# ndefilippis/SWRaytracing

Measured on AMD Instinct MI355X. Metric: packet-steps/sec @ 512² field, 1e6 packets; 1/2/4/8-GPU scaling, higher is better.
Workload: dtype f64

## Files before the change

### swraytracing_amd/csrc/swrt_bin.hpp

```cpp
#pragma once
#include <hip/hip_runtime.h>
#include <stdint.h>

#include "swrt_kernels.hpp"

namespace swrt {

struct BinGeom {
  double dx, px, py, inv_px, inv_py, inv_dx;
  int nx;
  int tile;
  int ntx;
};

__device__ __forceinline__ int tile_of(const BinGeom& g, double x, double y) {
  const int cx = fast_cell(x, g.inv_dx, g.nx);
  const int cy = fast_cell(y, g.inv_dx, g.nx);
  return (cx / g.tile) * g.ntx + (cy / g.tile);
}

constexpr int kMaxBins = 16384;
constexpr int kBinPerThread = 4;

__global__ void __launch_bounds__(256) bin_count_kernel(BinGeom g, const double* x, int64_t n,
                                                        int nbins, int* keys, int* counts) {
  extern __shared__ int hist[];
  for (int b = threadIdx.x; b < nbins; b += blockDim.x) hist[b] = 0;
  __syncthreads();
  const int64_t base = (int64_t)blockIdx.x * blockDim.x * kBinPerThread;
  for (int q = 0; q < kBinPerThread; ++q) {
    const int64_t p = base + (int64_t)q * blockDim.x + threadIdx.x;
    if (p < n) {
      const int key = tile_of(g, x[p], x[n + p]);
      keys[p] = key;
      atomicAdd(&hist[key], 1);
    }
  }
  __syncthreads();
  for (int b = threadIdx.x; b < nbins; b += blockDim.x) {
    const int c = hist[b];
    if (c) atomicAdd(&counts[b], c);
  }
}

constexpr int kOrderBuckets = 16;

__global__ void __launch_bounds__(1024) bin_scan_kernel(int* counts, int nbins, int* cursor,
                                                        int* starts, int64_t n, int* err, int* order = nullptr,
                                                        int lanes = 512) {
  __shared__ int part[1024];
  const int per = (nbins + 1023) / 1024;
  const int b0 = threadIdx.x * per;
  int s = 0;
  int neg = 0;
  for (int i = 0; i < per; ++i) {
    const int b = b0 + i;
    if (b < nbins) {
      const int c = counts[b];
      neg |= c < 0;
      s += c;
    }
  }
  part[threadIdx.x] = s;
  neg = __syncthreads_or(neg);
  for (int off = 1; off < 1024; off <<= 1) {
    const int v = threadIdx.x >= off ? part[threadIdx.x - off] : 0;
    __syncthreads();
    part[threadIdx.x] += v;
    __syncthreads();
  }
  if (neg || (int64_t)part[1023] != n) {
    for (int b = threadIdx.x; b < nbins; b += blockDim.x) {
      cursor[b] = (int)n;
      starts[b] = 0;
      counts[b] = 0;
    }
    if (threadIdx.x == 0) {
      starts[nbins] = 0;
      __hip_atomic_store(err, 1, __ATOMIC_RELAXED, __HIP_MEMORY_SCOPE_SYSTEM);
    }
    if (order != nullptr)
      for (int b = threadIdx.x; b < nbins; b += blockDim.x) order[b] = b;
    return;
  }
  int run = threadIdx.x ? part[threadIdx.x - 1] : 0;
  for (int i = 0; i < per; ++i) {
    const int b = b0 + i;
    if (b < nbins) {
      cursor[b] = run;
      starts[b] = run;
      run += counts[b];
      counts[b] = 0;
    }
  }
  if (threadIdx.x == 1023) starts[nbins] = part[1023];
  if (order == nullptr) return;
  __syncthreads();
  const int wave = threadIdx.x >> 6, lane = threadIdx.x & 63;
  if (nbins % 8 != 0) {
    for (int b = threadIdx.x; b < nbins; b += blockDim.x) order[b] = b;
    return;
  }
  if (wave >= 8) return;
  const int tpx = nbins / 8, base = wave * tpx;
  const uint64_t below = (1ull << lane) - 1;
  int cnt[kOrderBuckets];
#pragma unroll
  for (int v = 0; v < kOrderBuckets; ++v) cnt[v] = 0;
  for (int c0 = 0; c0 < tpx; c0 += 64) {
    const int i = c0 + lane;
    const int r = i < tpx ? min((starts[base + i + 1] - starts[base + i] + lanes - 1) / lanes, kOrderBuckets - 1) : -1;
#pragma unroll
    for (int v = 0; v < kOrderBuckets; ++v) cnt[v] += __popcll(__ballot(r == v));
  }
  int acc = 0;
#pragma unroll
  for (int v = kOrderBuckets - 1; v >= 0; --v) {
    const int c = cnt[v];
    cnt[v] = acc;
    acc += c;
  }
  for (int c0 = 0; c0 < tpx; c0 += 64) {
    const int i = c0 + lane;
    const int r = i < tpx ? min((starts[base + i + 1] - starts[base + i] + lanes - 1) / lanes, kOrderBuckets - 1) : -1;
#pragma unroll
    for (int v = 0; v < kOrderBuckets; ++v) {
      const uint64_t m = __ballot(r == v);
      if (r == v) order[base + cnt[v] + __popcll(m & below)] = base + i;
      cnt[v] += __popcll(m);
    }
  }
}

template <bool INDEX>
__global__ void __launch_bounds__(256) bin_scatter_kernel(const double* x, const double* k,
                                                          const int* perm, const int* keys, int64_t n,
                                                          int nbins, int* cursor, double* x2,
                                                          double* k2, int* perm2, int* src) {
  extern __shared__ int sh[];
  int* cnt = sh;
  int* base = sh + nbins;
  for (int b = threadIdx.x; b < nbins; b += blockDim.x) cnt[b] = 0;
  __syncthreads();
  const int64_t b0 = (int64_t)blockIdx.x * blockDim.x * kBinPerThread;
  int key[kBinPerThread], local[kBinPerThread];
#pragma unroll
  for (int q = 0; q < kBinPerThread; ++q) {
    const int64_t p = b0 + (int64_t)q * blockDim.x + threadIdx.x;
    key[q] = 0;
    local[q] = 0;
    if (p < n) {
      key[q] = keys[p];
      local[q] = atomicAdd(&cnt[key[q]], 1);
    }
  }
  __syncthreads();
  for (int b = threadIdx.x; b < nbins; b += blockDim.x) {
    const int c = cnt[b];
    if (c) base[b] = atomicAdd(&cursor[b], c);
  }
  __syncthreads();
#pragma unroll
  for (int q = 0; q < kBinPerThread; ++q) {
    const int64_t p = b0 + (int64_t)q * blockDim.x + threadIdx.x;
    if (p < n) {
      const int64_t d = (int64_t)base[key[q]] + local[q];
      if (d < 0 || d >= n) continue;
      if constexpr (INDEX) {
        src[d] = (int)p;
        continue;
      }
      x2[d] = x[p];
      x2[n + d] = x[n + p];
      k2[d] = k[p];
      k2[n + d] = k[n + p];
      perm2[d] = perm[p];
    }
  }
}

__global__ void iota_kernel(int* perm, int64_t n) {
  const int64_t p = (int64_t)blockIdx.x * blockDim.x + threadIdx.x;
  if (p < n) perm[p] = (int)p;
}

__global__ void unpermute_kernel(const double* x, const double* k, const int* perm, int64_t n, int64_t ld,
                                 double* xo, double* ko) {
  const int64_t p = (int64_t)blockIdx.x * blockDim.x + threadIdx.x;
  if (p >= n) return;
  const int64_t d = perm[p];
  xo[d] = x[p];
  xo[ld + d] = x[n + p];
  ko[d] = k[p];
  ko[ld + d] = k[n + p];
}

}
```

### swraytracing_amd/csrc/swrt_host_fields.hpp

```cpp
#pragma once
#include <vector>

#include "swrt_ctx.hpp"
#include "swrt_fft.hpp"
#include "swrt_kernels.hpp"
#include "swrt_xka.hpp"

namespace {

int ensure_scratch(swrt_ctx* c, size_t bytes) {
  if (c->scratch_bytes >= bytes) return SWRT_OK;
  c->scratch_bytes = 0;
  HIPCHK(c, c->scratch.alloc(bytes));
  c->scratch_bytes = bytes;
  return SWRT_OK;
}

int ensure_twiddles(swrt_ctx* c, int n) {
  if (c->tw_n == n) return SWRT_OK;
  if (c->tw) HIPCHK(c, hipDeviceSynchronize());
  std::vector<double2> h(n);
  for (int k = 0; k < n; ++k) {
    const long double th = -2.0L * 3.14159265358979323846264338327950288L * (long double)k / (long double)n;
    h[k] = make_double2((double)cosl(th), (double)sinl(th));
  }
  HIPCHK(c, c->tw.alloc(n));
  HIPCHK(c, hipMemcpyAsync(c->tw.get(), h.data(), sizeof(double2) * n, hipMemcpyHostToDevice,
                           c->stream));
  HIPCHK(c, hipStreamSynchronize(c->stream));
  c->tw_n = n;
  return SWRT_OK;
}

int ensure_slot(swrt_ctx* c, int slot, int64_t nx) {
  Slot& s = c->slot[slot];
  const int64_t npad = nx + kPadTot;
  if (s.nodes.get() && s.nx == nx) return SWRT_OK;
  if (s.nodes) HIPCHK(c, hipDeviceSynchronize());
  s.psi.reset();
  s.set = false;
  HIPCHK(c, s.nodes.alloc(kRec * npad * npad));
  s.nx = nx;
  s.npad = npad;
  return SWRT_OK;
}

int check_slot_args(swrt_ctx* c, int slot, int64_t nx) {
  if (!c) return SWRT_ERR_ARG;
  if (slot < 0 || slot >= SWRT_MAX_SLOTS) return fail(c, SWRT_ERR_ARG, "slot out of range");
  if (nx < 8 || nx > 4096 || (nx & 1)) return fail(c, SWRT_ERR_ARG, "nx must be even, 8..4096");
  return SWRT_OK;
}

FieldView view_of(const Slot& s) {
  FieldView v;
  v.nodes = s.nodes.get();
  v.nx = (int)s.nx;
  v.npad = (int)s.npad;
  v.dx = s.L / (double)s.nx;
  v.px = (double)s.nx;
  v.py = (double)s.ny_period;
  v.inv_px = 1.0 / v.px;
  v.inv_py = 1.0 / v.py;
  v.ipx = (int)s.nx;
  v.ipy = (int)s.ny_period;
  v.inv_dx = 1.0 / v.dx;
  return v;
}

int pack_slot(swrt_ctx* c, int slot, const double* dplanes, double shear) {
  Slot& s = c->slot[slot];
  const int64_t tot = s.npad * s.npad;
  hipLaunchKernelGGL(pack_nodes_kernel, dim3(nblocks(tot, 256)), dim3(256), 0, c->stream, dplanes,
                     (int)s.nx, (int)s.npad, shear, s.nodes.get());
  HIPCHK(c, hipGetLastError());
  return SWRT_OK;
}

int fft_group(const swrt_ctx* c, int n, int nvec, bool tin) {
  const int C = (c->qg_sep && c->n > 0) ? 1 : 2;
  if (C * (n / 4) > 1024 || nvec % (tin ? 8 * C : C) != 0) return 1;
  return C;
}

template <bool TIN>
void launch_fft(swrt_ctx* c, const double2* in, double2* out, int n, int logn, int nvec, int inverse) {
  if (n <= 1024) {
    const int C = fft_group(c, n, nvec, TIN);
    hipLaunchKernelGGL((fft_vec_kernel<TIN, 2>), dim3((unsigned)(nvec / C)), dim3(C * n / 4),
                       sizeof(double2) * C * (n + 1), c->stream, in, out, n, logn, c->tw.get(), inverse, nvec);
  } else
    hipLaunchKernelGGL((fft_vec_kernel<TIN, 1>), dim3((unsigned)nvec), dim3(128), sizeof(double2) * 2 * n, c->stream,
                       in, out, n, logn, c->tw.get(), inverse, nvec);
}

int run_fft_pass(swrt_ctx* c, double2* Z, int n, int nb, int inverse) {
  const int logn = ilog2(n);
  const int64_t nvec = (int64_t)n * nb;
  launch_fft<false>(c, Z, Z, n, logn, (int)nvec, inverse);
  HIPCHK(c, hipGetLastError());
  return SWRT_OK;
}

int run_transpose(swrt_ctx* c, const double2* in, double2* out, int n, int nb) {
  dim3 grid((n + 31) / 32, (n + 31) / 32, nb);
  hipLaunchKernelGGL(transpose_kernel, grid, dim3(32, 8), 0, c->stream, in, out, n);
  HIPCHK(c, hipGetLastError());
  return SWRT_OK;
}

int transform_2d(swrt_ctx* c, double2* Z, double2* out, int n, int nb, int inverse) {
  int rc;
  if ((rc = run_fft_pass(c, Z, n, nb, inverse))) return rc;
  const int64_t nvec = (int64_t)n * nb;
  if (nvec % 8) {
    if ((rc = run_transpose(c, Z, out, n, nb))) return rc;
    return run_fft_pass(c, out, n, nb, inverse);
  }
  const int logn = ilog2(n);
  launch_fft<true>(c, Z, out, n, logn, (int)nvec, inverse);
  HIPCHK(c, hipGetLastError());
  return SWRT_OK;
}

int inverse_2d(swrt_ctx* c, double2* Z, double2* out, int n, int nb) { return transform_2d(c, Z, out, n, nb, 1); }

int fields_from_halfplane(swrt_ctx* c, int slot, const double2* dfk, int n, int mode, double K_d2,
                          double kscale, double shear, int with_psi, double2* Z, double2* T, int sx, int sy) {
  int rc;
  const int64_t nn = (int64_t)n * n;
  const int nb = with_psi ? 4 : 3;
  Slot& s0 = c->slot[slot];
  if (!with_psi && n % 16 == 0 && 3 * 2 * n / 4 <= 1024 && (n / 2) % 8 == 0) {
    const int logn = ilog2(n);
    hipLaunchKernelGGL(spectra_rows_kernel, dim3((unsigned)n), dim3(3 * n / 4), sizeof(double2) * 3 * n, c->stream,
                       dfk, n, mode, K_d2, kscale, 0, sx, sy, logn, (const double2*)c->tw.get(), Z);
    HIPCHK(c, hipGetLastError());
    hipLaunchKernelGGL(fft_cols_pack_kernel<2>, dim3((unsigned)(n / 2)), dim3(3 * 2 * n / 4),
                       sizeof(double2) * 3 * 2 * (n + 1), c->stream, (const double2*)Z, n, logn,
                       (const double2*)c->tw.get(), (int)s0.npad, shear, s0.nodes.get());
    HIPCHK(c, hipGetLastError());
    s0.has_psi = false;
    s0.div_free = true;
    return SWRT_OK;
  }
  if (nb * n / 4 <= 1024 && ((int64_t)n * nb) % 8 == 0) {
    const int logn = ilog2(n);
    hipLaunchKernelGGL(spectra_rows_kernel, dim3((unsigned)n), dim3(nb * n / 4), sizeof(double2) * nb * n, c->stream,
                       dfk, n, mode, K_d2, kscale, with_psi, sx, sy, logn, (const double2*)c->tw.get(), Z);
    HIPCHK(c, hipGetLastError());
    launch_fft<true>(c, Z, T, n, logn, n * nb, 1);
    HIPCHK(c, hipGetLastError());
  } else {
    hipLaunchKernelGGL(spectra_kernel, dim3(nblocks(nn, 256)), dim3(256), 0, c->stream, dfk, n, mode,
                       K_d2, kscale, with_psi, Z, sx, sy);
    HIPCHK(c, hipGetLastError());
    if ((rc = inverse_2d(c, Z, T, n, nb))) return rc;
  }
  Slot& s = c->slot[slot];
  if (with_psi && !s.psi) HIPCHK(c, s.psi.alloc(nn));
  if (n % 16 == 0) {
    hipLaunchKernelGGL(pack_pairs_kernel, dim3(n / 16, n / 16), dim3(256), 0, c->stream, T, n, (int)s.npad, shear,
                       s.nodes.get());
    HIPCHK(c, hipGetLastError());
    if (with_psi) {
      hipLaunchKernelGGL(psi_plane_kernel, dim3(nblocks(nn, 256)), dim3(256), 0, c->stream, T + 3 * nn, s.psi.get(),
                         nn);
      HIPCHK(c, hipGetLastError());
    }
  } else {
    double* planes = reinterpret_cast<double*>(Z);
    hipLaunchKernelGGL(unpair_kernel, dim3(nblocks(nn, 256)), dim3(256), 0, c->stream, T, n, with_psi,
                       planes, with_psi ? s.psi.get() : nullptr);
    HIPCHK(c, hipGetLastError());
    if ((rc = pack_slot(c, slot, planes, shear))) return rc;
  }
  s.has_psi = with_psi != 0;
  s.div_free = true;
  return SWRT_OK;
}

struct FftScratch {
  double2 *Z, *T, *fk;
  double* raw;
};
FftScratch fft_scratch(swrt_ctx* c, size_t zb, int64_t nhalf) {
  char* base = c->scratch.get();
  return {(double2*)base, (double2*)(base + zb), (double2*)(base + 2 * zb),
          (double*)(base + 2 * zb + sizeof(double2) * nhalf)};
}

int g2k_launches(swrt_ctx* c, const double* raw, double2* Z, double2* T, double2* fk, int n) {
  const int64_t nn = (int64_t)n * n, nhalf = (int64_t)(n - 1) * (n / 2);
  hipLaunchKernelGGL(real_to_complex_kernel, dim3(nblocks(nn, 256)), dim3(256), 0, c->stream, raw, Z, nn);
  HIPCHK(c, hipGetLastError());
  if (int rc = transform_2d(c, Z, T, n, 1, 0)) return rc;
  hipLaunchKernelGGL(crop_half_kernel, dim3(nblocks(nhalf, 256)), dim3(256), 0, c->stream, T, n, fk);
  HIPCHK(c, hipGetLastError());
  return SWRT_OK;
}

int slot_set_done(swrt_ctx* c, int slot, double L, int64_t ny_period) {
  HIPCHK(c, hipStreamSynchronize(c->stream));
  Slot& s = c->slot[slot];
  s.L = L;
  s.ny_period = ny_period;
  s.set = true;
  s.wgen = ++c->slot_wgen;
  return SWRT_OK;
}

int xka_nodes_for(swrt_ctx* c, int64_t nx) {
  const int64_t npad = nx + kPadTot;
  if (c->xka.nx != nx) {
    c->xka.nx = 0;
    HIPCHK(c, c->xka.nodes.alloc(kXkaRec * npad * npad));
    c->xka.nx = nx;
  }
  return SWRT_OK;
}

int xka_pack(swrt_ctx* c, const double* dplanes, int64_t nx) {
  const int64_t npad = nx + kPadTot;
  hipLaunchKernelGGL(pack_xka_kernel, dim3(nblocks(npad * npad, 256)), dim3(256), 0, c->stream, dplanes, (int)nx,
                     (int)npad, c->xka.nodes.get());
  HIPCHK(c, hipGetLastError());
  return SWRT_OK;
}
}
```

### swraytracing_amd/csrc/swrt_kernels.hpp

```cpp
#pragma once
#include <hip/hip_runtime.h>
#include <stdint.h>

#include "swrt_share.hpp"

namespace swrt {

constexpr int kNT = 6;
constexpr int kPadLo = 2;
constexpr int kPadTot = 5;
constexpr int kRec = 6;

struct FieldView {
  const double* nodes;
  int nx;
  int npad;
  double dx;
  double px, py;
  double inv_px, inv_py;
  int ipx, ipy;
  double inv_dx;
};

__device__ __forceinline__ double div_rn(double a, double b, double rb) {
  const double q0 = a * rb;
  const double r = __builtin_fma(-q0, b, a);
  return __builtin_fma(r, rb, q0);
}

__device__ __forceinline__ double div_rn_z(double a, double b, double rb) {
  const double q0 = a * rb;
  const double r = __builtin_fma(q0, b, -a);
  return __builtin_fma(-r, rb, q0);
}

__device__ __forceinline__ double sqrt_rn_normal(double x) {
  const double y = __builtin_amdgcn_rsq(x);
  double g = x * y;
  double h = y * 0.5;
  const double r = __builtin_fma(-h, g, 0.5);
  g = __builtin_fma(g, r, g);
  double d = __builtin_fma(-g, g, x);
  h = __builtin_fma(h, r, h);
  g = __builtin_fma(d, h, g);
  d = __builtin_fma(-g, g, x);
  return __builtin_fma(d, h, g);
}

__device__ __forceinline__ double rcp_rn_normal(double b) {
  double y = __builtin_amdgcn_rcp(b);
  double e = __builtin_fma(-b, y, 1.0);
  y = __builtin_fma(y, e, y);
  e = __builtin_fma(-b, y, 1.0);
  y = __builtin_fma(y, e, y);
  const double r = __builtin_fma(-b, y, 1.0);
  return __builtin_fma(r, y, y);
}

__device__ __forceinline__ void drift_inc(double k, double l, double f2, double gH, double half, bool fast,
                                          double& hcx, double& hcy) {
  const double x = f2 + gH * (k * k + l * l);
  if (fast) {
    const double w = sqrt_rn_normal(x);
    const double rw = rcp_rn_normal(w);
    hcx = half * div_rn_z(gH * k, w, rw);
    hcy = half * div_rn_z(gH * l, w, rw);
  } else {
    const double w = sqrt(x);
    hcx = half * (gH * k / w);
    hcy = half * (gH * l / w);
  }
}

__device__ __forceinline__ void quot2_sqrt(double r, double n1, double n2, bool fast, double& q1, double& q2) {
  if (fast) {
    const double w = sqrt_rn_normal(r);
    const double rw = rcp_rn_normal(w);
    q1 = div_rn_z(n1, w, rw);
    q2 = div_rn_z(n2, w, rw);
  } else {
    const double w = sqrt(r);
    q1 = n1 / w;
    q2 = n2 / w;
  }
}

__host__ __device__ inline bool dispersion_fast(double f2) { return f2 >= 0x1p-767 && f2 < 0x1p+1000; }

__global__ void __launch_bounds__(256) check_arith_kernel(int64_t n, uint64_t seed,
                                                          unsigned long long* mismatches) {
  const int64_t p = (int64_t)blockIdx.x * blockDim.x + threadIdx.x;
  if (p >= n) return;
  uint64_t s = seed ^ (0x9E3779B97F4A7C15ull * (uint64_t)(p + 1));
  auto nxt = [&]() {
    s ^= s << 13; s ^= s >> 7; s ^= s << 17;
    return s;
  };
  auto rnd = [&](int lo, int hi) {
    const uint64_t m = nxt() & ((1ull << 52) - 1);
    const int e = lo + (int)(nxt() % (uint64_t)(hi - lo + 1));
    return __longlong_as_double((long long)(((uint64_t)(e + 1023) << 52) | m));
  };
  unsigned bad[3] = {0, 0, 0};
  for (int it = 0; it < 16; ++it) {
    const double x = rnd(-767, 1023);
    if (__double_as_longlong(sqrt_rn_normal(x)) != __double_as_longlong(sqrt(x))) ++bad[0];
    const double w = rnd(-383, 511);
    if (__double_as_longlong(rcp_rn_normal(w)) != __double_as_longlong(1.0 / w)) ++bad[1];
    const double f2 = rnd(-60, 60), gH = rnd(-30, 30);
    const double k = (nxt() & 1 ? -1.0 : 1.0) * rnd(-40, 40), l = (nxt() & 1 ? -1.0 : 1.0) * rnd(-40, 40);
    double hx, hy, gx, gy;
    drift_inc(k, l, f2, gH, 0.5, true, hx, hy);
    drift_inc(k, l, f2, gH, 0.5, false, gx, gy);
    if (__double_as_longlong(hx) != __double_as_longlong(gx) || __double_as_longlong(hy) != __double_as_longlong(gy))
      ++bad[2];
  }
  for (int q = 0; q < 3; ++q)
    if (bad[q]) atomicAdd(&mismatches[q], (unsigned long long)bad[q]);
}

__device__ __forceinline__ int cvt_i32_sat(double v) {
  int c;
  asm("v_cvt_i32_f64 %0, %1" : "=v"(c) : "v"(v));
  return c;
}

__device__ __forceinline__ int cell_frac(double x, double dx, double inv_dx, double period,
                                         double inv_period, int iperiod, int nx, double& a) {
  const double q = div_rn(x, dx, inv_dx);
  const double r = div_rn(q, period, inv_period);
  const double xl = q - floor(r) * period;
  const double fl = floor(xl);
  a = (1.0 + xl) - (1.0 + fl);
  int c = cvt_i32_sat(fl);
  c = (unsigned)c > (unsigned)iperiod ? 0 : c;
  c = (int)min((unsigned)c, (unsigned)(c - nx));
  c = (int)min((unsigned)c, (unsigned)(c - nx));
  if (iperiod >= 3 * nx) c %= nx;
  return c;
}

template <int D>
__device__ __forceinline__ double div_const(double x) {
  constexpr int A = D < 0 ? -D : D;
  static_assert(A >= 1 && A <= 5, "divisor");
  double q;
  if constexpr (A == 1 || A == 2 || A == 4) {
    q = x * (1.0 / (double)A);
  } else {
    constexpr double R = 1.0 / (double)A;
    const double q0 = x * R;
    const double r = __builtin_fma(-q0, (double)A, x);
    q = __builtin_fma(r, R, q0);
  }
  return D < 0 ? -q : q;
}

constexpr int odd_part(int d) { return d < 0 ? odd_part(-d) : (d % 2 == 0 ? odd_part(d / 2) : d); }
constexpr double pow2_sign_inv(int d) {
  return d < 0 ? -pow2_sign_inv(-d) : (d % 2 == 0 ? 0.5 * pow2_sign_inv(d / 2) : 1.0);
}
template <int I>
constexpr double kScale() {
  double c = 1.0;
  for (int j = -2; j <= 3; ++j)
    if (j != I) c *= pow2_sign_inv(j - I);
  return c;
}

template <int I, int J>
__device__ __forceinline__ double wstep(double w, const double* t) {
  if constexpr (I == J) {
    return w;
  } else {
    return div_const<odd_part(J - I)>(w * t[J + 2]);
  }
}

template <int I>
__device__ __forceinline__ double lagrange_wi(const double* t) {
  double w = 1.0;
  w = wstep<I, -2>(w, t);
  w = wstep<I, -1>(w, t);
  w = wstep<I, 0>(w, t);
  w = wstep<I, 1>(w, t);
  w = wstep<I, 2>(w, t);
  w = wstep<I, 3>(w, t);
  constexpr double S = kScale<I>();
  return S == 1.0 ? w : w * S;
}

__device__ __forceinline__ void lagrange_w(double a, double bump, double w[kNT]) {
  double t[kNT];
#pragma unroll
  for (int j = -2; j <= 3; ++j) t[j + 2] = (a - (double)j) + bump;
  w[0] = lagrange_wi<-2>(t);
  w[1] = lagrange_wi<-1>(t);
  w[2] = lagrange_wi<0>(t);
  w[3] = lagrange_wi<1>(t);
  w[4] = lagrange_wi<2>(t);
  w[5] = lagrange_wi<3>(t);
}

__device__ __forceinline__ int fast_cell(double x, double inv_dx, int nx) {
  const double q = floor(x * inv_dx);
  int c = (q > -1073741824.0 && q < 1073741824.0) ? (int)q : 0;
  c %= nx;
  return c < 0 ? c + nx : c;
}

struct Stencil {
  int ic, jc;
  double wx[kNT], wy[kNT];
};

__device__ __forceinline__ void stencil_at(const FieldView& fv, double x, double y, double bump,
                                           Stencil& s) {
  double ax, ay;
  s.ic = cell_frac(x, fv.dx, fv.inv_dx, fv.px, fv.inv_px, fv.ipx, fv.nx, ax);
  s.jc = cell_frac(y, fv.dx, fv.inv_dx, fv.py, fv.inv_py, fv.ipy, fv.nx, ay);
  lagrange_w(ax, bump, s.wx);
  lagrange_w(ay, bump, s.wy);
}

template <bool TWO>
__device__ __forceinline__ void gather6(const double* nodes0, const double* nodes1, int npad,
                                        const Stencil& s, double o0[kRec], double o1[kRec]) {
#pragma unroll
  for (int f = 0; f < kRec; ++f) { o0[f] = -0.0; o1[f] = -0.0; }
  const size_t off = ((size_t)s.ic * npad + s.jc) * kRec;
#pragma unroll
  for (int i = 0; i < kNT; ++i) {
    const size_t ro = off + (size_t)i * npad * kRec;
    const double2* r0 = reinterpret_cast<const double2*>(nodes0 + ro);
    const double2* r1 = reinterpret_cast<const double2*>(nodes1 + ro);
#pragma unroll
    for (int j = 0; j < kNT; ++j) {
      const double wij = s.wx[i] * s.wy[j];
      const double2 a0 = r0[3 * j + 0], a1 = r0[3 * j + 1], a2 = r0[3 * j + 2];
      o0[0] = o0[0] + wij * a0.x; o0[1] = o0[1] + wij * a0.y;
      o0[2] = o0[2] + wij * a1.x; o0[3] = o0[3] + wij * a1.y;
      o0[4] = o0[4] + wij * a2.x; o0[5] = o0[5] + wij * a2.y;
      if constexpr (TWO) {
        const double2 b0 = r1[3 * j + 0], b1 = r1[3 * j + 1], b2 = r1[3 * j + 2];
        o1[0] = o1[0] + wij * b0.x; o1[1] = o1[1] + wij * b0.y;
        o1[2] = o1[2] + wij * b1.x; o1[3] = o1[3] + wij * b1.y;
        o1[4] = o1[4] + wij * b2.x; o1[5] = o1[5] + wij * b2.y;
      }
    }
  }
}

__device__ __forceinline__ void interp6(const FieldView& fv, double x, double y, double bump,
                                        double out[kRec]) {
  Stencil s;
  stencil_at(fv, x, y, bump, s);
  double dummy[kRec];
  gather6<false>(fv.nodes, fv.nodes, fv.npad, s, out, dummy);
}

template <bool FMA>
__device__ __forceinline__ double madd(double acc, double w, double v) {
  if constexpr (FMA)
    return __builtin_fma(w, v, acc);
  else
    return acc + w * v;
}

template <bool TWO, bool FMA = false>
__device__ __forceinline__ void gather6_lean(const double* nodes0, const double* nodes1, int npad,
                                             const Stencil& s, double o0[kRec], double o1[kRec]) {
#pragma unroll
  for (int f = 0; f < kRec; ++f) { o0[f] = -0.0; o1[f] = -0.0; }
  const size_t off = ((size_t)s.ic * npad + s.jc) * kRec;
#pragma unroll
  for (int i = 0; i < kNT; ++i) {
    const size_t ro = off + (size_t)i * npad * kRec;
    const double2* r0 = reinterpret_cast<const double2*>(nodes0 + ro);
    const double2* r1 = reinterpret_cast<const double2*>(nodes1 + ro);
#pragma unroll
    for (int j = 0; j < kNT; ++j) {
      const double wij = s.wx[i] * s.wy[j];
      const double2 a0 = r0[3 * j + 0], a1 = r0[3 * j + 1], a2 = r0[3 * j + 2];
      o0[0] = madd<FMA>(o0[0], wij, a0.x); o0[1] = madd<FMA>(o0[1], wij, a0.y);
      o0[2] = madd<FMA>(o0[2], wij, a1.x); o0[3] = madd<FMA>(o0[3], wij, a1.y);
      o0[4] = madd<FMA>(o0[4], wij, a2.x); o0[5] = madd<FMA>(o0[5], wij, a2.y);
      if constexpr (TWO) {
        const double2 b0 = r1[3 * j + 0], b1 = r1[3 * j + 1], b2 = r1[3 * j + 2];
        o1[0] = madd<FMA>(o1[0], wij, b0.x); o1[1] = madd<FMA>(o1[1], wij, b0.y);
        o1[2] = madd<FMA>(o1[2], wij, b1.x); o1[3] = madd<FMA>(o1[3], wij, b1.y);
        o1[4] = madd<FMA>(o1[4], wij, b2.x); o1[5] = madd<FMA>(o1[5], wij, b2.y);
      }
      __builtin_amdgcn_sched_barrier(0);
    }
  }
}

template <bool TWO>
__device__ __forceinline__ void eval_flow_t(const FieldView& f0, const FieldView& f1, double alpha,
                                            double x, double y, double bump, double I[kRec]) {
  Stencil s;
  stencil_at(f0, x, y, bump, s);
  double J[kRec];
  gather6<TWO>(f0.nodes, f1.nodes, f0.npad, s, I, J);
  if constexpr (TWO) {
    const double oma = 1 - alpha;
#pragma unroll
    for (int q = 0; q < kRec; ++q) I[q] = oma * I[q] + alpha * J[q];
  }
}

__device__ __forceinline__ void eval_flow(const FieldView& f0, const FieldView& f1, int nslots,
                                          double alpha, double x, double y, double bump,
                                          double I[kRec]) {
  if (nslots == 2)
    eval_flow_t<true>(f0, f1, alpha, x, y, bump, I);
  else
    eval_flow_t<false>(f0, f1, alpha, x, y, bump, I);
}

constexpr int kMaxIntervals = 4;

struct StepArgs {
  FieldView f0, f1;
  int nslots;
  double* x;
  double* k;
  int64_t n;
  double dt, half, f2, gH;
  int fastdisp;
  double alpha0, dalpha;
  int64_t s0;
  int nsteps;
  double bump;
  int64_t save_every;
  double* hist_x;
  double* hist_k;
  int64_t frame0;
  const int* perm;
};


template <bool TWO>
__global__ void __launch_bounds__(256) leapfrog_kernel(StepArgs a) {
  const int64_t p = xcd_block(blockIdx.x, gridDim.x) * blockDim.x + threadIdx.x;
  if (p >= a.n) return;
  double x0 = a.x[p], y0 = a.x[a.n + p];
  double k0 = a.k[p], l0 = a.k[a.n + p];
  double hcx, hcy;
  drift_inc(k0, l0, a.f2, a.gH, a.half, a.fastdisp, hcx, hcy);
  for (int s = 0; s < a.nsteps; ++s) {
    const int64_t sg = a.s0 + s;
    const double x1 = x0 + hcx;
    const double y1 = y0 + hcy;
    double I[kRec];
    eval_flow_t<TWO>(a.f0, a.f1, a.alpha0 + (double)sg * a.dalpha, x1, y1, a.bump, I);
    const double x2 = x1 + a.dt * I[0];
    const double y2 = y1 + a.dt * I[1];
    const double k2 = k0 - a.dt * (I[2] * k0 + I[4] * l0);
    const double l2 = l0 - a.dt * (I[3] * k0 + I[5] * l0);
    drift_inc(k2, l2, a.f2, a.gH, a.half, a.fastdisp, hcx, hcy);
    x0 = x2 + hcx;
    y0 = y2 + hcy;
    k0 = k2;
    l0 = l2;
    if (a.hist_x != nullptr && ((sg + 1) % a.save_every) == 0) {
      const int64_t fr = a.frame0 + (sg + 1) / a.save_every - 1;
      double* hx = a.hist_x + fr * 2 * a.n;
      double* hk = a.hist_k + fr * 2 * a.n;
      const int64_t o = a.perm[p];
      hx[o] = x0; hx[a.n + o] = y0;
      hk[o] = k0; hk[a.n + o] = l0;
    }
  }
  a.x[p] = x0; a.x[a.n + p] = y0;
  a.k[p] = k0; a.k[a.n + p] = l0;
}

__global__ void __launch_bounds__(256) eval_kernel(FieldView f0, FieldView f1, int nslots,
                                                   double alpha, double bump, const double* x,
                                                   const double* y, int64_t n, double* out) {
  const int64_t p = (int64_t)blockIdx.x * blockDim.x + threadIdx.x;
  if (p >= n) return;
  double I[kRec];
  eval_flow(f0, f1, nslots, alpha, x[p], y[p], bump, I);
#pragma unroll
  for (int q = 0; q < kRec; ++q) out[(int64_t)q * n + p] = I[q];
}

__global__ void __launch_bounds__(256) interp1_kernel(const double* F, int nx, double pyF,
                                                      double inv_py, double dx,
                                                      double dy, double bump, const double* x,
                                                      const double* y, int64_t n, double* out) {
  const int64_t p = (int64_t)blockIdx.x * blockDim.x + threadIdx.x;
  if (p >= n) return;
  const double px = (double)nx;
  double ax, ay;
  const int ic = cell_frac(x[p], dx, 1.0 / dx, px, 1.0 / px, nx, nx, ax);
  const int jc = cell_frac(y[p], dy, 1.0 / dy, pyF, inv_py, (int)pyF, nx, ay);
  double wx[kNT], wy[kNT];
  lagrange_w(ax, bump, wx);
  lagrange_w(ay, bump, wy);
  double FI = 0.0;
#pragma unroll
  for (int i = 0; i < kNT; ++i) {
    int ig = ic + i - 2;
    ig = ig < 0 ? ig + nx : (ig >= nx ? ig - nx : ig);
#pragma unroll
    for (int j = 0; j < kNT; ++j) {
      int jg = jc + j - 2;
      jg = jg < 0 ? jg + nx : (jg >= nx ? jg - nx : jg);
      FI = FI + wx[i] * wy[j] * F[ig + (size_t)nx * jg];
    }
  }
  out[p] = FI;
}

__global__ void pack_nodes_kernel(const double* planes, int nx, int npad, double shear,
                                  double* nodes) {
  const int64_t idx = (int64_t)blockIdx.x * blockDim.x + threadIdx.x;
  const int64_t tot = (int64_t)npad * npad;
  if (idx >= tot) return;
  const int ip = (int)idx / npad, jp = (int)idx % npad;
  int ig = ip - kPadLo, jg = jp - kPadLo;
  ig = ((ig % nx) + nx) % nx;
  jg = ((jg % nx) + nx) % nx;
  const int64_t plane = (int64_t)nx * nx;
  const int64_t src = ig + (int64_t)nx * jg;
  double* dst = nodes + idx * kRec;
#pragma unroll
  for (int f = 0; f < kRec; ++f) dst[f] = planes[f * plane + src] + (f == 0 ? shear : 0.0);
}

__global__ void unpack_nodes_kernel(const double* nodes, int nx, int npad, double* planes) {
  const int64_t idx = (int64_t)blockIdx.x * blockDim.x + threadIdx.x;
  const int64_t plane = (int64_t)nx * nx;
  if (idx >= plane) return;
  const int ig = (int)idx % nx, jg = (int)idx / nx;
  const double* src = nodes + ((int64_t)(ig + kPadLo) * npad + (jg + kPadLo)) * kRec;
#pragma unroll
  for (int f = 0; f < kRec; ++f) planes[f * plane + idx] = src[f];
}

}
```

### swraytracing_amd/csrc/swrt_tile.hpp

```cpp
#pragma once
#include <hip/hip_runtime.h>
#include <stdint.h>

#include "swrt_kernels.hpp"

namespace swrt {

struct TileArgs {
  StepArgs s;
  double* x_out;
  double* k_out;
  int* perm_out;
  const int* starts;
  const int* order;
  int ntx;
  int* next_keys;
  int* next_counts;
  int sort_cells;
  const int* src;
  double sort_lead;
  TileShare sh;
  int ivmode;
  int nint;
  const double* ivn[kMaxIntervals + 1];
  double ivdt[kMaxIntervals];
};

__device__ __forceinline__ const double* iv_nodes(const TileArgs& ta, int i) {
  const double* p = ta.ivn[0];
#pragma unroll
  for (int j = 1; j <= kMaxIntervals; ++j)
    if (i == j) p = ta.ivn[j];
  return p;
}
__device__ __forceinline__ double iv_dt(const TileArgs& ta, int i) {
  double d = ta.ivdt[0];
#pragma unroll
  for (int j = 1; j < kMaxIntervals; ++j)
    if (i == j) d = ta.ivdt[j];
  return d;
}

__device__ __forceinline__ int wg_work_range(const int* starts, const int* order, int64_t n, const TileShare& sh,
                                             int& pbeg, int& pend) {
  int tile = share_slot(sh, (int)blockIdx.x);
  if (order != nullptr) tile = order[tile];
  const int nn = (int)n;
  pbeg = min(max(starts[tile], 0), nn);
  pend = min(max(starts[tile + 1], pbeg), nn);
  return tile;
}
__device__ __forceinline__ int wg_work_range(const int* starts, int64_t n, int& pbeg, int& pend) {
  TileShare sh;
  sh.ntiles = (int)gridDim.x;
  return wg_work_range(starts, nullptr, n, sh, pbeg, pend);
}

__device__ __forceinline__ int wg_work(const TileArgs& ta, int& pbeg, int& pend) {
  return wg_work_range(ta.starts, ta.order, ta.s.n, ta.sh, pbeg, pend);
}

__device__ __forceinline__ int ring_diff(int a, int b, int n) {
  int d = a - b;
  if (d >= n / 2) d -= n;
  if (d < -n / 2) d += n;
  return d;
}

__device__ __forceinline__ int b128_lane_rank(int lane) {
  const int h = lane & 32, t = lane & 31;
  int k;
  if (t < 4) k = t;
  else if (t < 12) k = 16 + (t - 4);
  else if (t < 16) k = 4 + (t - 12);
  else if (t < 20) k = 24 + (t - 16);
  else if (t < 28) k = 8 + (t - 20);
  else k = t;
  return h + k;
}

template <bool TWO>
struct Tap6 {
  double2 a0, a1, a2, b0, b1, b2;
};
template <bool TWO, int WN>
__device__ __forceinline__ void tap6_read(const double2* p, int e, Tap6<TWO>& t) {
  t.a0 = p[0 * WN + e];
  t.a1 = p[1 * WN + e];
  t.a2 = p[2 * WN + e];
  if constexpr (TWO) {
    t.b0 = p[3 * WN + e];
    t.b1 = p[4 * WN + e];
    t.b2 = p[5 * WN + e];
  }
}
template <bool TWO, int W, int WN>
__device__ __forceinline__ void gather6_lds(const double2* lds, int node0, const Stencil& s,
                                            double o0[kRec], double o1[kRec]) {
#pragma unroll
  for (int f = 0; f < kRec; ++f) { o0[f] = -0.0; o1[f] = -0.0; }
  const double2* p = lds + node0;
  double wx[kNT], wy[kNT];
#pragma unroll
  for (int q = 0; q < kNT; ++q) {
    wx[q] = s.wx[q];
    wy[q] = s.wy[q];
    asm volatile("" : "+v"(wx[q]));
    asm volatile("" : "+v"(wy[q]));
  }
  if constexpr (TWO) {
#pragma unroll
    for (int i = 0; i < kNT; ++i) {
#pragma unroll
      for (int j = 0; j < kNT; ++j) {
        const int e = i * W + j;
        const double wij = wx[i] * wy[j];
        const double2 a0 = p[0 * WN + e], a1 = p[1 * WN + e], a2 = p[2 * WN + e];
        o0[0] = o0[0] + wij * a0.x; o0[1] = o0[1] + wij * a0.y;
        o0[2] = o0[2] + wij * a1.x; o0[3] = o0[3] + wij * a1.y;
        o0[4] = o0[4] + wij * a2.x; o0[5] = o0[5] + wij * a2.y;
        const double2 b0 = p[3 * WN + e], b1 = p[4 * WN + e], b2 = p[5 * WN + e];
        o1[0] = o1[0] + wij * b0.x; o1[1] = o1[1] + wij * b0.y;
        o1[2] = o1[2] + wij * b1.x; o1[3] = o1[3] + wij * b1.y;
        o1[4] = o1[4] + wij * b2.x; o1[5] = o1[5] + wij * b2.y;
      }
    }
    return;
  }
  Tap6<TWO> cur, nxt;
  tap6_read<TWO, WN>(p, 0, cur);
#pragma unroll
  for (int t = 0; t < kNT * kNT; ++t) {
    const int i = t / kNT, j = t % kNT;
    if (t + 1 < kNT * kNT) tap6_read<TWO, WN>(p, ((t + 1) / kNT) * W + (t + 1) % kNT, nxt);
    if constexpr (!TWO) __builtin_amdgcn_sched_barrier(0);
    const double wij = wx[i] * wy[j];
    o0[0] = o0[0] + wij * cur.a0.x; o0[1] = o0[1] + wij * cur.a0.y;
    o0[2] = o0[2] + wij * cur.a1.x; o0[3] = o0[3] + wij * cur.a1.y;
    o0[4] = o0[4] + wij * cur.a2.x; o0[5] = o0[5] + wij * cur.a2.y;
    if constexpr (TWO) {
      o1[0] = o1[0] + wij * cur.b0.x; o1[1] = o1[1] + wij * cur.b0.y;
      o1[2] = o1[2] + wij * cur.b1.x; o1[3] = o1[3] + wij * cur.b1.y;
      o1[4] = o1[4] + wij * cur.b2.x; o1[5] = o1[5] + wij * cur.b2.y;
    }
    if constexpr (!TWO) __builtin_amdgcn_sched_barrier(0);
    if (t + 1 < kNT * kNT) cur = nxt;
  }
}

template <bool TWO>
struct Tap5 {
  double2 a0, a1, c, b0, b1;
};
template <bool TWO, int WN>
__device__ __forceinline__ void tap5_read(const double2* p, int e, Tap5<TWO>& t) {
  t.a0 = p[0 * WN + e];
  t.a1 = p[1 * WN + e];
  if constexpr (TWO) {
    t.c = p[2 * WN + e];
    t.b0 = p[3 * WN + e];
    t.b1 = p[4 * WN + e];
  } else {
    t.c.x = reinterpret_cast<const double*>(p + 2 * WN + e)[0];
  }
}
template <bool TWO, int W, int WN, bool FMA = false, int PF = 1>
__device__ __forceinline__ void gather5_lds(const double2* lds, int node0, const Stencil& s,
                                            double o0[kRec], double o1[kRec]) {
  static_assert(PF >= 1 && PF <= 4, "prefetch depth");
  constexpr int NTAP = kNT * kNT;
#pragma unroll
  for (int f = 0; f < 5; ++f) { o0[f] = -0.0; o1[f] = -0.0; }
  const double2* p = lds + node0;
  double wx[kNT], wy[kNT];
#pragma unroll
  for (int q = 0; q < kNT; ++q) {
    wx[q] = s.wx[q];
    wy[q] = s.wy[q];
    asm volatile("" : "+v"(wx[q]));
    asm volatile("" : "+v"(wy[q]));
  }
  Tap5<TWO> ring[PF + 1];
#pragma unroll
  for (int t = 0; t < PF; ++t) tap5_read<TWO, WN>(p, (t / kNT) * W + t % kNT, ring[t]);
#pragma unroll
  for (int t = 0; t < NTAP; ++t) {
    const int i = t / kNT, j = t % kNT;
    if (t + PF < NTAP) tap5_read<TWO, WN>(p, ((t + PF) / kNT) * W + (t + PF) % kNT, ring[(t + PF) % (PF + 1)]);
    __builtin_amdgcn_sched_barrier(0);
    const Tap5<TWO>& cur = ring[t % (PF + 1)];
    const double wij = wx[i] * wy[j];
    o0[0] = madd<FMA>(o0[0], wij, cur.a0.x); o0[1] = madd<FMA>(o0[1], wij, cur.a0.y);
    o0[2] = madd<FMA>(o0[2], wij, cur.a1.x); o0[3] = madd<FMA>(o0[3], wij, cur.a1.y);
    o0[4] = madd<FMA>(o0[4], wij, cur.c.x);
    if constexpr (TWO) {
      o1[0] = madd<FMA>(o1[0], wij, cur.b0.x); o1[1] = madd<FMA>(o1[1], wij, cur.b0.y);
      o1[2] = madd<FMA>(o1[2], wij, cur.b1.x); o1[3] = madd<FMA>(o1[3], wij, cur.b1.y);
      o1[4] = madd<FMA>(o1[4], wij, cur.c.y);
    }
    __builtin_amdgcn_sched_barrier(0);
  }
  o0[5] = -o0[2];
  o1[5] = -o1[2];
}

template <bool TWO, int T, int M, int NT, int WS = T + 5 + 2 * M, bool V5 = false>
__device__ __forceinline__ void stage_window_regs(const FieldView& f0, const FieldView& f1, int ox, int oy,
                                                  double2* win) {
  constexpr int W = T + 5 + 2 * M;
  constexpr int WN = W * WS;
  const int nx = f0.nx, npad = f0.npad;
  for (int e = threadIdx.x; e < W * W; e += NT) {
    const int wi = e / W, wj = e % W;
    int gx = (ox - M - 2 + wi) % nx; gx += gx < 0 ? nx : 0;
    int gy = (oy - M - 2 + wj) % nx; gy += gy < 0 ? nx : 0;
    const size_t src = ((size_t)(gx + kPadLo) * npad + (gy + kPadLo)) * kRec;
    const int d = wi * WS + wj;
    const double2* s0 = reinterpret_cast<const double2*>(f0.nodes + src);
    if constexpr (V5 && TWO) {
      const double2* s1 = reinterpret_cast<const double2*>(f1.nodes + src);
      const double2 a0 = s0[0], a1 = s0[1], a2 = s0[2], b0 = s1[0], b1 = s1[1], b2 = s1[2];
      win[0 * WN + d] = a0;
      win[1 * WN + d] = a1;
      win[2 * WN + d] = make_double2(a2.x, b2.x);
      win[3 * WN + d] = b0;
      win[4 * WN + d] = b1;
    } else {
      win[0 * WN + d] = s0[0];
      win[1 * WN + d] = s0[1];
      win[2 * WN + d] = s0[2];
      if constexpr (TWO) {
        const double2* s1 = reinterpret_cast<const double2*>(f1.nodes + src);
        win[3 * WN + d] = s1[0];
        win[4 * WN + d] = s1[1];
        win[5 * WN + d] = s1[2];
      }
    }
  }
}

#ifdef SWRT_PHASE_TIMING
__device__ unsigned long long swrt_phase_dbg[16384 * 8];
#define SWRT_STAMP(slot)                                                            \
  do {                                                                              \
    if (tid == 0) swrt_phase_dbg[blockIdx.x * 8 + (slot)] = __builtin_amdgcn_s_memrealtime(); \
  } while (0)
#else
#define SWRT_STAMP(slot) \
  do {                   \
  } while (0)
#endif

#ifndef SWRT_TILE_MIN_WAVES
#define SWRT_TILE_MIN_WAVES 4
#endif

template <bool TWO, int T, int M, int NT, bool V5 = false, bool FMA = false, int PF = 1,
          int MINW = SWRT_TILE_MIN_WAVES>
__global__ void __launch_bounds__(NT, MINW) tile_leapfrog_kernel(TileArgs ta) {
  static_assert(!FMA || V5, "the FMA gather exists for the five-sum window only");
  constexpr int W = T + 5 + 2 * M;
  constexpr int WS = W + ((12 - W % 16) + 16) % 16;
  constexpr int WNP = W * WS;
  constexpr int NCH = TWO ? (V5 ? 5 : 6) : 3;
  constexpr int NB = T * T + 1;
  constexpr int MAXB = 2 * NT;
  __shared__ double2 win[NCH * WNP];
  __shared__ int hist[NB];
  __shared__ int kr[MAXB];
  __shared__ int order[MAXB];
  __shared__ int nbr[9];
#ifdef SWRT_PHASE_TIMING
  __shared__ int nfall;
  __shared__ unsigned simds;
#endif

  const StepArgs& a = ta.s;
  const int tid = threadIdx.x;
  int pbeg, pend;
  const int tile = wg_work(ta, pbeg, pend);
  const int tx = tile / ta.ntx, ty = tile % ta.ntx;
  const int nx = a.f0.nx, npad = a.f0.npad;
  const int ox = tx * T, oy = ty * T;
  if (tid < 9) nbr[tid] = 0;
#ifdef SWRT_PHASE_TIMING
  if (tid == 0) nfall = 0;
  if (tid == 0) simds = 0;
#endif
  SWRT_STAMP(0);
#ifdef SWRT_PHASE_TIMING
  if (tid == 0) {
    unsigned hw, xcc;
    asm volatile("s_getreg_b32 %0, hwreg(HW_REG_HW_ID)" : "=s"(hw));
    asm volatile("s_getreg_b32 %0, hwreg(HW_REG_XCC_ID)" : "=s"(xcc));
    swrt_phase_dbg[blockIdx.x * 8 + 7] = ((unsigned long long)xcc << 32) | hw;
    swrt_phase_dbg[blockIdx.x * 8 + 6] = (unsigned long long)(pend - pbeg);
  }
  __syncthreads();
  if ((tid & 63) == 0) {
    unsigned hw;
    asm volatile("s_getreg_b32 %0, hwreg(HW_REG_HW_ID)" : "=s"(hw));
    atomicOr(&simds, ((hw >> 4) & 3u) << (2 * (tid >> 6)));
  }
  __syncthreads();
  if (tid == 0) swrt_phase_dbg[blockIdx.x * 8 + 6] |= (unsigned long long)simds << 32;
#endif

  const int lane_rank = b128_lane_rank(tid & 63);
  const int nint = ta.ivmode ? ta.nint : 1;
  for (int ivl = 0; ivl < nint; ++ivl) {
  FieldView fa = a.f0, fb = a.f1;
  if (ta.ivmode) {
    fa.nodes = iv_nodes(ta, ivl);
    fb.nodes = iv_nodes(ta, ivl + 1);
  }
  const double dt = ta.ivmode ? iv_dt(ta, ivl) : a.dt;
  const double half = ta.ivmode ? 0.5 * dt : a.half;
  const bool first = ivl == 0;
  const double* xin = first ? a.x : ta.x_out;
  const double* kin = first ? a.k : ta.k_out;
  const int* pin = first ? a.perm : ta.perm_out;
  const int sortc = first ? ta.sort_cells : 0;
  const int* srcp = first ? ta.src : nullptr;
  int* nkeys = ivl == nint - 1 ? ta.next_keys : nullptr;
  const int64_t sbase = a.s0 + (int64_t)ivl * a.nsteps;
  if (!first) __syncthreads();

  stage_window_regs<TWO, T, M, NT, WS, V5>(fa, fb, ox, oy, win);
  if (!sortc) {
    __syncthreads();
    SWRT_STAMP(1);
  }
  for (int b0 = pbeg; b0 < pend; b0 += MAXB) {
    const int nb = min(MAXB, pend - b0);
    if (sortc) {
    for (int h = tid; h < NB; h += NT) hist[h] = 0;
    __syncthreads();
    if (b0 == pbeg) SWRT_STAMP(1);
    for (int i = tid; i < nb; i += NT) {
      const int64_t p = srcp ? srcp[b0 + i] : b0 + i;
      double xs = xin[p], ys = xin[a.n + p];
      if (ta.sort_lead != 0.0) {
        const double kx = kin[p], ky = kin[a.n + p];
        const double s = ta.sort_lead * a.gH / sqrt(a.f2 + a.gH * (kx * kx + ky * ky));
        xs += s * kx;
        ys += s * ky;
      }
      const int ic = fast_cell(xs, a.f0.inv_dx, nx);
      const int jc = fast_cell(ys, a.f0.inv_dx, nx);
      const int dx_ = min(max(ring_diff(ic, ox, nx), 0), T - 1);
      const int dy_ = min(max(ring_diff(jc, oy, nx), 0), T - 1);
      int key;
      if constexpr (T == 16) {
        key = (dx_ >= 0 && dx_ < T && dy_ >= 0 && dy_ < T)
                  ? ((dy_ & 1) | ((dx_ & 1) << 1) | ((dy_ & 2) << 1) | ((dx_ & 2) << 2) |
                     ((dy_ & 4) << 2) | ((dx_ & 4) << 3) | ((dy_ & 8) << 3) | ((dx_ & 8) << 4))
                  : T * T;
      } else {
        key = 0;
#pragma unroll
        for (int b = 0; (1 << b) < T; ++b) key |= (((dy_ >> b) & 1) << (2 * b)) | (((dx_ >> b) & 1) << (2 * b + 1));
      }
      const int r = atomicAdd(&hist[key], 1);
      kr[i] = (key << 16) | r;
    }
    __syncthreads();
    if (tid < 64) {
      constexpr int PER = (NB + 63) / 64;
      int loc[PER];
      int sum = 0;
#pragma unroll
      for (int q = 0; q < PER; ++q) {
        const int h = tid * PER + q;
        loc[q] = h < NB ? hist[h] : 0;
        sum += loc[q];
      }
      int incl = sum;
#pragma unroll
      for (int off = 1; off < 64; off <<= 1) {
        const int v = __shfl_up(incl, off, 64);
        if (tid >= off) incl += v;
      }
      int run = incl - sum;
#pragma unroll
      for (int q = 0; q < PER; ++q) {
        const int h = tid * PER + q;
        if (h < NB) hist[h] = run;
        run += loc[q];
      }
    }
    __syncthreads();
    for (int i = tid; i < nb; i += NT) {
      const int v = kr[i];
      order[hist[v >> 16] + (v & 0xffff)] = srcp ? srcp[b0 + i] : b0 + i;
    }
    __syncthreads();
    }
    if (b0 == pbeg) SWRT_STAMP(2);

    for (int r0 = tid & ~63; r0 < nb; r0 += NT) {
      const int r = r0 + lane_rank;
      if (r >= nb) continue;
      const int64_t pi = sortc ? order[r] : b0 + r;
      const int64_t po = b0 + r;
      double x0 = xin[pi], y0 = xin[a.n + pi];
      double k0 = kin[pi], l0 = kin[a.n + pi];
      const int orig = pin[pi];
      double hcx, hcy;
      drift_inc(k0, l0, a.f2, a.gH, half, a.fastdisp, hcx, hcy);
      double sgd = (double)(ta.ivmode ? (int64_t)0 : sbase);
      for (int st = 0; st < a.nsteps; ++st) {
        const int64_t sg = sbase + st;
        const double alpha = a.alpha0 + sgd * a.dalpha;
        sgd = sgd + 1.0;
        const double x1 = x0 + hcx;
        const double y1 = y0 + hcy;
        Stencil sc;
        stencil_at(a.f0, x1, y1, a.bump, sc);
        const int dx_ = ring_diff(sc.ic, ox, nx), dy_ = ring_diff(sc.jc, oy, nx);
        double I[kRec], J[kRec];
        const bool inwin = dx_ >= -M && dx_ < T + M && dy_ >= -M && dy_ < T + M;
#ifdef SWRT_PHASE_TIMING
        if (!inwin) atomicAdd(&nfall, 1);
#endif
        if (inwin) {
          if constexpr (V5)
            gather5_lds<TWO, WS, WNP, FMA, PF>(win, (dx_ + M) * WS + (dy_ + M), sc, I, J);
          else
            gather6_lds<TWO, WS, WNP>(win, (dx_ + M) * WS + (dy_ + M), sc, I, J);
        } else {
          gather6_lean<TWO, FMA>(fa.nodes, fb.nodes, npad, sc, I, J);
        }
        if constexpr (TWO) {
          const double oma = 1 - alpha;
#pragma unroll
          for (int q = 0; q < (V5 ? 5 : kRec); ++q) I[q] = madd<FMA>(oma * I[q], alpha, J[q]);
          if constexpr (V5) I[5] = -I[2];
        }
        const double x2 = x1 + dt * I[0];
        const double y2 = y1 + dt * I[1];
        const double k2 = k0 - dt * (I[2] * k0 + I[4] * l0);
        const double l2 = l0 - dt * (I[3] * k0 + I[5] * l0);
        drift_inc(k2, l2, a.f2, a.gH, half, a.fastdisp, hcx, hcy);
        x0 = x2 + hcx;
        y0 = y2 + hcy;
        k0 = k2;
        l0 = l2;
        if (a.hist_x != nullptr && ((sg + 1) % a.save_every) == 0) {
          const int64_t fr = a.frame0 + (sg + 1) / a.save_every - 1;
          double* hx = a.hist_x + fr * 2 * a.n;
          double* hk = a.hist_k + fr * 2 * a.n;
          hx[orig] = x0; hx[a.n + orig] = y0;
          hk[orig] = k0; hk[a.n + orig] = l0;
        }
      }
      ta.x_out[po] = x0; ta.x_out[a.n + po] = y0;
      ta.k_out[po] = k0; ta.k_out[a.n + po] = l0;
      ta.perm_out[po] = orig;
      if (nkeys != nullptr) {
        const int ic = fast_cell(x0, a.f0.inv_dx, nx);
        const int jc = fast_cell(y0, a.f0.inv_dx, nx);
        const int ntx_ = ta.ntx;
        const int ntx2 = ic / T, nty2 = jc / T;
        nkeys[po] = ntx2 * ntx_ + nty2;
        const int ddx = ring_diff(ntx2, tx, ntx_), ddy = ring_diff(nty2, ty, ntx_);
        if (ddx != 0 || ddy != 0) {
          atomicAdd(&nbr[4], -1);
          if (ddx >= -1 && ddx <= 1 && ddy >= -1 && ddy <= 1)
            atomicAdd(&nbr[(ddx + 1) * 3 + (ddy + 1)], 1);
          else
            atomicAdd(&ta.next_counts[ntx2 * ntx_ + nty2], 1);
        }
      }
    }
    __syncthreads();
    if (b0 == pbeg) SWRT_STAMP(3);
  }
  }
  if (ta.next_keys != nullptr) {
    __syncthreads();
    const int v = tid < 9 ? nbr[tid] + (tid == 4 ? pend - pbeg : 0) : 0;
    if (v != 0) {
      const int n_ = ta.ntx;
      const int gx = ((tx + tid / 3 - 1) % n_ + n_) % n_, gy = ((ty + tid % 3 - 1) % n_ + n_) % n_;
      atomicAdd(&ta.next_counts[gx * n_ + gy], v);
    }
  }
  SWRT_STAMP(4);
#ifdef SWRT_PHASE_TIMING
  __syncthreads();
  if (tid == 0) swrt_phase_dbg[blockIdx.x * 8 + 5] = (unsigned long long)nfall;
#endif
}

}
```

Measured before the change: 25.65 billion.

## Trim per-step cell indexing, window test, and binning scan/atomic overheads

```diff
diff --git a/swraytracing_amd/csrc/swrt_bin.hpp b/swraytracing_amd/csrc/swrt_bin.hpp
--- a/swraytracing_amd/csrc/swrt_bin.hpp
+++ b/swraytracing_amd/csrc/swrt_bin.hpp
@@ -48,9 +48,10 @@
 __global__ void __launch_bounds__(1024) bin_scan_kernel(int* counts, int nbins, int* cursor,
                                                         int* starts, int64_t n, int* err, int* order = nullptr,
                                                         int lanes = 512) {
-  __shared__ int part[1024];
+  __shared__ int wtot[16];
   const int per = (nbins + 1023) / 1024;
   const int b0 = threadIdx.x * per;
+  const int wave = threadIdx.x >> 6, lane = threadIdx.x & 63;
   int s = 0;
   int neg = 0;
   for (int i = 0; i < per; ++i) {
@@ -61,15 +62,24 @@
       s += c;
     }
   }
-  part[threadIdx.x] = s;
+  int incl = s;
+#pragma unroll
+  for (int off = 1; off < 64; off <<= 1) {
+    const int v = __shfl_up(incl, off, 64);
+    if (lane >= off) incl += v;
+  }
+  if (lane == 63) wtot[wave] = incl;
   neg = __syncthreads_or(neg);
-  for (int off = 1; off < 1024; off <<= 1) {
-    const int v = threadIdx.x >= off ? part[threadIdx.x - off] : 0;
-    __syncthreads();
-    part[threadIdx.x] += v;
-    __syncthreads();
-  }
-  if (neg || (int64_t)part[1023] != n) {
+  const int wt = lane < 16 ? wtot[lane] : 0;
+  int wincl = wt;
+#pragma unroll
+  for (int off = 1; off < 16; off <<= 1) {
+    const int v = __shfl_up(wincl, off, 64);
+    if (lane >= off) wincl += v;
+  }
+  const int total = __shfl(wincl, 15, 64);
+  incl += __shfl(wincl - wt, wave, 64);
+  if (neg || (int64_t)total != n) {
     for (int b = threadIdx.x; b < nbins; b += blockDim.x) {
       cursor[b] = (int)n;
       starts[b] = 0;
@@ -83,7 +93,7 @@
       for (int b = threadIdx.x; b < nbins; b += blockDim.x) order[b] = b;
     return;
   }
-  int run = threadIdx.x ? part[threadIdx.x - 1] : 0;
+  int run = incl - s;
   for (int i = 0; i < per; ++i) {
     const int b = b0 + i;
     if (b < nbins) {
@@ -93,10 +103,9 @@
       counts[b] = 0;
     }
   }
-  if (threadIdx.x == 1023) starts[nbins] = part[1023];
+  if (threadIdx.x == 1023) starts[nbins] = total;
   if (order == nullptr) return;
   __syncthreads();
-  const int wave = threadIdx.x >> 6, lane = threadIdx.x & 63;
   if (nbins % 8 != 0) {
     for (int b = threadIdx.x; b < nbins; b += blockDim.x) order[b] = b;
     return;
@@ -143,16 +152,23 @@
   for (int b = threadIdx.x; b < nbins; b += blockDim.x) cnt[b] = 0;
   __syncthreads();
   const int64_t b0 = (int64_t)blockIdx.x * blockDim.x * kBinPerThread;
+  const int lane = threadIdx.x & 63;
+  const uint64_t upto = (2ull << lane) - 1;
   int key[kBinPerThread], local[kBinPerThread];
 #pragma unroll
   for (int q = 0; q < kBinPerThread; ++q) {
     const int64_t p = b0 + (int64_t)q * blockDim.x + threadIdx.x;
-    key[q] = 0;
-    local[q] = 0;
-    if (p < n) {
-      key[q] = keys[p];
-      local[q] = atomicAdd(&cnt[key[q]], 1);
-    }
+    key[q] = p < n ? keys[p] : -1;
+    const int prev = __shfl_up(key[q], 1, 64);
+    const bool head = lane == 0 || prev != key[q];
+    const uint64_t heads = __ballot(head);
+    const int hl = 63 - __clzll((long long)(heads & upto));
+    const uint64_t above = heads & ~upto;
+    const int next = above ? __ffsll((unsigned long long)above) - 1 : 64;
+    int base_q = 0;
+    if (head && key[q] >= 0) base_q = atomicAdd(&cnt[key[q]], next - lane);
+    local[q] = __shfl(base_q, hl, 64) + (lane - hl);
+    if (key[q] < 0) key[q] = 0;
   }
   __syncthreads();
   for (int b = threadIdx.x; b < nbins; b += blockDim.x) {
diff --git a/swraytracing_amd/csrc/swrt_host_fields.hpp b/swraytracing_amd/csrc/swrt_host_fields.hpp
--- a/swraytracing_amd/csrc/swrt_host_fields.hpp
+++ b/swraytracing_amd/csrc/swrt_host_fields.hpp
@@ -65,6 +65,9 @@
   v.ipx = (int)s.nx;
   v.ipy = (int)s.ny_period;
   v.inv_dx = 1.0 / v.dx;
+  const auto pow2 = [](int p) { return p > 0 && (p & (p - 1)) == 0; };
+  v.inv_exact = pow2(v.ipx) && pow2(v.ipy);
+  v.ywrap1 = v.ipy == v.nx;
   return v;
 }
 
diff --git a/swraytracing_amd/csrc/swrt_kernels.hpp b/swraytracing_amd/csrc/swrt_kernels.hpp
--- a/swraytracing_amd/csrc/swrt_kernels.hpp
+++ b/swraytracing_amd/csrc/swrt_kernels.hpp
@@ -20,6 +20,8 @@
   double inv_px, inv_py;
   int ipx, ipy;
   double inv_dx;
+  int inv_exact;
+  int ywrap1;
 };
 
 __device__ __forceinline__ double div_rn(double a, double b, double rb) {
@@ -125,19 +127,34 @@
   return c;
 }
 
-__device__ __forceinline__ int cell_frac(double x, double dx, double inv_dx, double period,
-                                         double inv_period, int iperiod, int nx, double& a) {
+__device__ __forceinline__ double cell_quot(double x, double dx, double inv_dx, double inv_period, double& r) {
   const double q = div_rn(x, dx, inv_dx);
-  const double r = div_rn(q, period, inv_period);
+  r = q * inv_period;
+  return q;
+}
+__device__ __forceinline__ double cell_quot_fix(double q, double r, double period, double inv_period) {
+  return __builtin_fma(__builtin_fma(-r, period, q), inv_period, r);
+}
+__device__ __forceinline__ int cell_tail(double q, double r, double period, int iperiod, int nx, double& a,
+                                         bool one_wrap) {
   const double xl = q - floor(r) * period;
   const double fl = floor(xl);
   a = (1.0 + xl) - (1.0 + fl);
   int c = cvt_i32_sat(fl);
   c = (unsigned)c > (unsigned)iperiod ? 0 : c;
   c = (int)min((unsigned)c, (unsigned)(c - nx));
+  if (one_wrap) return c;
   c = (int)min((unsigned)c, (unsigned)(c - nx));
   if (iperiod >= 3 * nx) c %= nx;
   return c;
+}
+__device__ __forceinline__ int cell_frac(double x, double dx, double inv_dx, double period,
+                                         double inv_period, int iperiod, int nx, double& a,
+                                         bool exact_inv = false, bool one_wrap = false) {
+  double r;
+  const double q = cell_quot(x, dx, inv_dx, inv_period, r);
+  if (!exact_inv) r = cell_quot_fix(q, r, period, inv_period);
+  return cell_tail(q, r, period, iperiod, nx, a, one_wrap);
 }
 
 template <int D>
@@ -168,12 +185,41 @@
   return c;
 }
 
+
+template <int I>
+constexpr bool fold_scale() { return I != 1; }
+template <int I>
+constexpr int fold_step() {
+  for (int j = -2; j <= 3; ++j)
+    if (j != I && odd_part(j - I) != 1) return j;
+  return 99;
+}
+template <int I>
+constexpr int last_step() { return I == 3 ? 2 : 3; }
+constexpr double abs_c(double v) { return v < 0 ? -v : v; }
+
+template <int A>
+__device__ __forceinline__ double div_const_scaled(double x, double S) {
+  static_assert(A == 3 || A == 5, "divisor");
+  const double R = (1.0 / (double)A) * S;
+  const double q0 = x * R;
+  const double r = __builtin_fma(-q0, (double)A / S, x);
+  return __builtin_fma(r, R, q0);
+}
+
 template <int I, int J>
 __device__ __forceinline__ double wstep(double w, const double* t) {
   if constexpr (I == J) {
     return w;
   } else {
-    return div_const<odd_part(J - I)>(w * t[J + 2]);
+    constexpr double S = kScale<I>();
+    constexpr bool neg = fold_scale<I>() && S < 0 && J == last_step<I>();
+    static_assert(!neg || odd_part(J - I) == 1, "the sign rides on a step without a Markstein correction");
+    const double x = neg ? (-w) * t[J + 2] : w * t[J + 2];
+    if constexpr (fold_scale<I>() && J == fold_step<I>())
+      return div_const_scaled<odd_part(J - I)>(x, abs_c(S));
+    else
+      return div_const<odd_part(J - I)>(x);
   }
 }
 
@@ -187,7 +233,7 @@
   w = wstep<I, 2>(w, t);
   w = wstep<I, 3>(w, t);
   constexpr double S = kScale<I>();
-  return S == 1.0 ? w : w * S;
+  return (fold_scale<I>() || S == 1.0) ? w : w * S;
 }
 
 __device__ __forceinline__ void lagrange_w(double a, double bump, double w[kNT]) {
@@ -217,8 +263,16 @@
 __device__ __forceinline__ void stencil_at(const FieldView& fv, double x, double y, double bump,
                                            Stencil& s) {
   double ax, ay;
-  s.ic = cell_frac(x, fv.dx, fv.inv_dx, fv.px, fv.inv_px, fv.ipx, fv.nx, ax);
-  s.jc = cell_frac(y, fv.dx, fv.inv_dx, fv.py, fv.inv_py, fv.ipy, fv.nx, ay);
+  double rx, ry;
+  const double qx = cell_quot(x, fv.dx, fv.inv_dx, fv.inv_px, rx);
+  const double qy = cell_quot(y, fv.dx, fv.inv_dx, fv.inv_py, ry);
+  if (!fv.inv_exact) {
+    rx = cell_quot_fix(qx, rx, fv.px, fv.inv_px);
+    ry = cell_quot_fix(qy, ry, fv.py, fv.inv_py);
+    asm volatile("" : "+v"(rx), "+v"(ry));
+  }
+  s.ic = cell_tail(qx, rx, fv.px, fv.nx, fv.nx, ax, true);
+  s.jc = cell_tail(qy, ry, fv.py, fv.ipy, fv.nx, ay, fv.ywrap1 != 0);
   lagrange_w(ax, bump, s.wx);
   lagrange_w(ay, bump, s.wy);
 }
diff --git a/swraytracing_amd/csrc/swrt_tile.hpp b/swraytracing_amd/csrc/swrt_tile.hpp
--- a/swraytracing_amd/csrc/swrt_tile.hpp
+++ b/swraytracing_amd/csrc/swrt_tile.hpp
@@ -282,6 +282,7 @@
   const int tx = tile / ta.ntx, ty = tile % ta.ntx;
   const int nx = a.f0.nx, npad = a.f0.npad;
   const int ox = tx * T, oy = ty * T;
+  const int oxm = ((ox - M) % nx + nx) % nx, oym = ((oy - M) % nx + nx) % nx;
   if (tid < 9) nbr[tid] = 0;
 #ifdef SWRT_PHASE_TIMING
   if (tid == 0) nfall = 0;
@@ -417,17 +418,18 @@
         const double y1 = y0 + hcy;
         Stencil sc;
         stencil_at(a.f0, x1, y1, a.bump, sc);
-        const int dx_ = ring_diff(sc.ic, ox, nx), dy_ = ring_diff(sc.jc, oy, nx);
+        const int d0 = sc.ic - oxm, d1 = sc.jc - oym;
+        const unsigned ux = min((unsigned)d0, (unsigned)(d0 + nx)), uy = min((unsigned)d1, (unsigned)(d1 + nx));
         double I[kRec], J[kRec];
-        const bool inwin = dx_ >= -M && dx_ < T + M && dy_ >= -M && dy_ < T + M;
+        const bool inwin = max(ux, uy) < (unsigned)(T + 2 * M);
 #ifdef SWRT_PHASE_TIMING
         if (!inwin) atomicAdd(&nfall, 1);
 #endif
         if (inwin) {
           if constexpr (V5)
-            gather5_lds<TWO, WS, WNP, FMA, PF>(win, (dx_ + M) * WS + (dy_ + M), sc, I, J);
+            gather5_lds<TWO, WS, WNP, FMA, PF>(win, (int)(ux * WS + uy), sc, I, J);
           else
-            gather6_lds<TWO, WS, WNP>(win, (dx_ + M) * WS + (dy_ + M), sc, I, J);
+            gather6_lds<TWO, WS, WNP>(win, (int)(ux * WS + uy), sc, I, J);
         } else {
           gather6_lean<TWO, FMA>(fa.nodes, fb.nodes, npad, sc, I, J);
         }
```

Result: faster. 26.01 billion (median of 6 runs) (+1.4%).
